# khimansusinha/Distributed-sorting-with-fault-tolerance

Measured on AMD Instinct MI355X. Metric: sorted keys/sec (int32, 2^30 keys), higher is better.
Workload: dtype int32; 1 GPU; C2-style single-GPU sort of 1073741824 uniform int32 keys (BASELINE metric size); tile 8192 keys, 0 merge passes; keys=1073741824, parallelism=1 GPU

## Files before the change

### distributed-sorting-with-fault-tolerance_amd/csrc/dsort_bucket.h

```cpp
#pragma once
#include <hip/hip_runtime.h>
#include <stdint.h>

#include <type_traits>

#include "dsort_internal.h"

namespace dsort {
namespace bk {

constexpr int BK_T = 1024;
constexpr int BK_MAXB = 1024;
constexpr int BK_OS = 32;
constexpr int BK_CHUNK = 16;
constexpr int BK_CSEG = 16;

template <typename T> struct Geo;
template <> struct Geo<int32_t> { static constexpr int KPT = 16; };
constexpr int BK_KPT64 = 6;
template <> struct Geo<int64_t> { static constexpr int KPT = BK_KPT64; };
typedef int bk_v4i __attribute__((ext_vector_type(4)));
typedef long long bk_v2l __attribute__((ext_vector_type(2)));
template <typename T> struct BkIds {
    static constexpr bool ON = sizeof(T) == 8;
// ... 58 lines not shown
template <typename T>
__device__ __forceinline__ int bucket_of(const typename Comp<T>::C *spl, int BP,
                                         const typename Comp<T>::C &c) {
    int lo = 0;
    for (int st = BP >> 1; st >= 1; st >>= 1) lo += Comp<T>::lt(spl[lo + st - 1], c) ? st : 0;
    return lo;
}

constexpr int BK_SLOTB = 11;
constexpr int BK_SLOTS = 1 << BK_SLOTB;

struct BkMap {
    uint64_t ulo;
    uint32_t sh;
    uint32_t mode;
    uint64_t invn;
    uint32_t ids;
    uint32_t hot;
    uint32_t one;
    uint32_t ad;
    uint32_t r2s;
    uint32_t r2lo;
    uint32_t r2sh;
};
constexpr int BK_R2 = 256;
constexpr int BK_R2_BITS = 8;
constexpr uint32_t BK_R2_IMPLIED = 0x4000u;
constexpr size_t BK_MAP_BYTES = 64 + 4 * BK_R2;
static_assert(sizeof(BkMap) <= 64, "the refined table sits 64 bytes into the map");
__host__ __device__ __forceinline__ const uint32_t *bk_tab2(const BkMap *m) {
    return reinterpret_cast<const uint32_t *>(reinterpret_cast<const char *>(m) + 64);
}
constexpr uint32_t BK_PACKED_R2 = 0xFFFFFu;
constexpr uint32_t BK_R2_FLAG = 0x4000u;

template <typename T>
__device__ __forceinline__ uint32_t bucket_runs_hint(uint32_t nasc, uint32_t ndup, int nsp) {
    if (nsp < 16) return 0;
    const uint32_t pairs = (uint32_t)(nsp - 1);
    (void)ndup;
    return (8 * nasc >= 7 * pairs || 8 * nasc <= pairs) ? 1u : 0u;
}
template <bool RANK>
__device__ __forceinline__ uint32_t bucket_bump(uint32_t *hist, int b, bool act) {
    const uint64_t am = __ballot(act);
    if (!am) return 0u;
    const int lane = (int)(threadIdx.x & 63), first = (int)__ffsll((long long)am) - 1;
// ... 179 lines not shown
        if (in == 3) return bucket_onekey<T>(spl, lo, hi, key, c);
        while (lo < hi) {
            const int mid = (lo + hi) >> 1;
            if (Comp<T>::lt(spl[mid], c)) lo = mid + 1;
            else hi = mid;
        }
        return lo;
    }
    if constexpr (!ADP) {
        if (ONE && tab2 && (r & BK_R2_FLAG))
            return refine_pick<T>(spl, tab2[refine_sub(m->r2lo, m->r2sh, (int32_t)key)], key, c);
    }
    int lo = (int)(r & 0x3FFF), hi = (int)(r >> 16);
    if (ONE && (r & 0x8000)) return bucket_onekey<T>(spl, lo, hi, key, c);
    while (lo < hi) {
        const int mid = (lo + hi) >> 1;
        if (Comp<T>::lt(spl[mid], c)) lo = mid + 1;
        else hi = mid;
    }
    return lo;
}

template <typename T>
__global__ void __launch_bounds__(BK_MAXB) bucket_slotmap_kernel(const typename Comp<T>::C *__restrict__ spl,
                                                                  int B, uint64_t n, BkMap *__restrict__ out) {
    using CT = Comp<T>;
    using U = typename CT::U;
    __shared__ uint32_t cnt[2][BK_SLOTS];
    __shared__ uint32_t crowd[2];
    const int j = threadIdx.x, nsp = B - 1;
    for (int i = j; i < 2 * BK_SLOTS; i += blockDim.x) cnt[i / BK_SLOTS][i % BK_SLOTS] = 0;
    if (j < 2) crowd[j] = 0;
    __shared__ uint32_t dup;
    __shared__ uint32_t nasc, ndup;
    if (j == 0) dup = nasc = ndup = 0;
    __syncthreads();
    if (j + 1 < nsp) {
        if (CT::idx_of(spl[j]) < CT::idx_of(spl[j + 1])) atomicAdd(&nasc, 1u);
        if (CT::key_of(spl[j]) == CT::key_of(spl[j + 1])) atomicAdd(&ndup, 1u);
    }
    const uint64_t invn = ((uint64_t)1 << 48) / (n > 0 ? n : 1);
    BkMap mm[2] = {{0, (uint32_t)(CT::KB - BK_SLOTB), 0, invn, 0, 0}, {0, 0, 1, invn, 0, 0}};
    if constexpr (!CT::ADAPT) {
        constexpr uint32_t AD_MIX = 8;
        __shared__ uint32_t tot[3][BK_SLOTS], dst[3][BK_SLOTS];
        __shared__ uint32_t cost[3];
        for (int i = j; i < 3 * BK_SLOTS; i += blockDim.x) tot[i / BK_SLOTS][i % BK_SLOTS] = dst[i / BK_SLOTS][i % BK_SLOTS] = 0;
        if (j < 3) cost[j] = 0;
// ... 17 lines not shown
                if (first) atomicAdd(&dst[q][sl[q]], 1u);
            }
        }
        __syncthreads();
        for (int i = j; i < 3 * BK_SLOTS; i += blockDim.x)
            if (dst[i / BK_SLOTS][i % BK_SLOTS] >= 2) atomicMax(&cost[i / BK_SLOTS], tot[i / BK_SLOTS][i % BK_SLOTS]);
        __syncthreads();
        __shared__ uint32_t r2slot, cost2;
        __shared__ BkMap rm;
        if (j == 0) {
            r2slot = ~0u;
            cost2 = 0;
        }
        __syncthreads();
        const int qa = cost[2] < cost[1] ? 2 : 1;
        if (cost[0] > AD_MIX && cost[qa] > AD_MIX)
            for (int i = j; i < BK_SLOTS; i += blockDim.x)
                if (dst[0][i] >= 2 && tot[0][i] == cost[0]) atomicMin(&r2slot, (uint32_t)i);
        __syncthreads();
        if (r2slot != ~0u)
            for (int i = j; i < BK_SLOTS; i += blockDim.x)
                if ((uint32_t)i != r2slot && dst[0][i] >= 2) atomicMax(&cost2, tot[0][i]);
        __syncthreads();
        const bool refine = r2slot != ~0u && cost2 <= cost[qa];
        const bool fixed = cost[0] <= AD_MIX || refine;
        if (j == 0) {
            if (!refine) r2slot = ~0u;
            BkMap r = fixed ? am[0] : am[qa];
            r.ad = r.ulo != 0 || r.mode != 0 || r.sh != (uint32_t)(CT::KB - BK_SLOTB) ? 1u : 0u;
            r.ids = 0;
            r.hot = bucket_runs_hint<T>(nasc, ndup, nsp);
            r.one = r.ad ? 1u : (ndup != 0);
            r.r2s = r.r2lo = r.r2sh = 0;
            if (r2slot != ~0u) {
                uint32_t a = 0, z = 0;
                for (int k = 0; k < nsp; ++k) {
                    const uint32_t sk = slot_mode<T, BK_SLOTB, 0, false>(am[0], CT::key_of(spl[k]));
                    a += sk < r2slot;
                    z += sk <= r2slot;
                }
                uint64_t us0 = 0;
                (void)slot_first<T, BK_SLOTB>(am[0], r2slot, us0);
                const uint32_t k0 = CT::flip(CT::key_of(spl[a])), hi = CT::flip(CT::key_of(spl[z - 1 - (z - a) / 32]));
                const uint32_t lo = r2slot > 0 && k0 > (uint32_t)us0 ? k0 - 1 : k0;
                const uint32_t rr = hi - lo;
                const int bits = rr == 0 ? 0 : 32 - __builtin_clz(rr);
                r.r2s = r2slot + 1;
                r.r2lo = lo;
                r.r2sh = (uint32_t)(bits > BK_R2_BITS ? bits - BK_R2_BITS : 0);
                r.one = 1;
                static_assert(BK_R2 == 1 << BK_R2_BITS, "sub-slots");
// ... 16 lines not shown
                    const uint32_t mid = (lo + hi) >> 1;
                    if (CT::lt(spl[mid], cc)) lo = mid + 1;
                    else hi = mid;
                }
                return lo;
            };
            (void)BPl;
            const uint32_t c_lo = s2 == 0 ? 0u : below(us), c_hi = has_next ? below(ue) : (uint32_t)nsp;
            for (int i = j; i < BK_R2; i += blockDim.x) {
                uint32_t c0 = c_lo, c1 = c_hi;
                if (i > 0) {
                    const uint64_t u = (uint64_t)rm.r2lo + ((uint64_t)i << rm.r2sh);
                    c0 = has_next && u >= ue ? c_hi : (u > 0xFFFFFFFFull ? c_hi : below(u));
                }
                if (i + 1 < BK_R2) {
                    const uint64_t u = (uint64_t)rm.r2lo + ((uint64_t)(i + 1) << rm.r2sh);
                    c1 = has_next && u >= ue ? c_hi : (u > 0xFFFFFFFFull ? c_hi : below(u));
                }
                c0 = c0 < c_lo ? c_lo : c0;
                const bool one = c1 >= c0 + 2 && CT::key_of(spl[c0]) == CT::key_of(spl[c1 - 1]);
                const bool implied = rm.r2sh == 0 && i > 0 && i + 1 < BK_R2;
                tab[i] = c0 | (implied ? BK_R2_IMPLIED : 0u) | (uint32_t)one << 15 | c1 << 16;
            }
        }
        return;
    }
    if (nsp >= 1) {
        const U lo = CT::flip(CT::key_of(spl[0])), hi = CT::flip(CT::key_of(spl[nsp - 1]));
        const U r = hi - lo;
        const int bits = r == 0 ? 0 : (int)(sizeof(U) * 8) - (sizeof(U) == 8 ? __builtin_clzll((uint64_t)r)
                                                                               : __builtin_clz((uint32_t)r));
        mm[0] = BkMap{(uint64_t)lo, (uint32_t)(bits > BK_SLOTB ? bits - BK_SLOTB : 0), 0, invn, 0, 0};
        mm[1] = BkMap{(uint64_t)lo, 0, 1, invn, 0, 0};
    }
    __syncthreads();
    if (j > 0 && j < nsp && CT::key_of(spl[j]) == CT::key_of(spl[j - 1])) dup = 1;
    if (j < nsp && (j == 0 || CT::key_of(spl[j]) != CT::key_of(spl[j - 1]))) {
        const T k = CT::key_of(spl[j]);
        atomicAdd(&cnt[0][slot_at<T>(mm[0], k)], 1u);
        atomicAdd(&cnt[1][slot_at<T>(mm[1], k)], 1u);
    }
    __syncthreads();
    for (int i = j; i < 2 * BK_SLOTS; i += blockDim.x) atomicMax(&crowd[i / BK_SLOTS], cnt[i / BK_SLOTS][i % BK_SLOTS]);
    __syncthreads();
    if (j == 0) {
        BkMap r = crowd[1] < crowd[0] ? mm[1] : mm[0];
// ... 81 lines not shown

constexpr uint64_t BK_CUS = 256;
template <typename T>
__host__ __forceinline__ int bucket_wg_subs(uint64_t n) {
    const uint64_t sub = (uint64_t)BK_T * Geo<T>::KPT;
    const uint64_t v = n / (2048 * sub);
    const int cap = v < 4 ? 4 : (v > 16 ? 16 : (int)v);
    if (cap > 4) {
        const uint64_t nsub = (n + sub - 1) / sub;
        int best = cap;
        uint64_t bcost = ~0ull;
        for (int s = cap; s >= (cap + 1) / 2; --s) {
            const uint64_t rounds = ((nsub + s - 1) / s + BK_CUS - 1) / BK_CUS;
            if (rounds * s < bcost) {
                bcost = rounds * s;
                best = s;
            }
        }
        return best;
    }
    return cap;
}

template <typename T, bool AD = false>
__global__ void __launch_bounds__(BK_T, 2) bucket_hist_kernel(const T *__restrict__ in, uint64_t n,
                                                              const typename Comp<T>::C *__restrict__ spl_g,
                                                              const BkMap *__restrict__ map, int B, int BP,
                                                              int subs, uint32_t *__restrict__ counts,
                                                              uint64_t ioff, uint32_t *__restrict__ ids) {
    using CT = Comp<T>;
    constexpr bool ADP = CT::ADAPT || AD;
    constexpr int KPT = Geo<T>::KPT, SUB = BK_T * KPT;
    static_assert(!BkIds<T>::ON || KPT % BkIds<T>::PER_WORD == 0, "bucket ids: whole words per thread");
    __shared__ typename CT::C spl[BK_MAXB + 1];
    __shared__ uint32_t rng[BK_SLOTS];
    const BkMap m = *map;
    if (!ADP && m.ad) return;
    __shared__ uint32_t hist[BK_MAXB];
    __shared__ uint32_t tab2[ADP ? 1 : BK_R2];
    load_splitters<T>(spl_g, BP, spl);
    for (int b = threadIdx.x; b < B; b += BK_T) hist[b] = 0;
    if (!ADP && m.r2s)
        for (int i = threadIdx.x; i < BK_R2; i += BK_T) tab2[i] = bk_tab2(map)[i];
    __syncthreads();
    build_slots<T, false, BK_SLOTB, ADP>(spl, BP, m, rng);
    __syncthreads();
    const uint64_t g0 = (uint64_t)blockIdx.x * subs * SUB;
    T nxt[KPT];
    load_sub<T, KPT, false>(in, g0 + threadIdx.x, n, g0 + SUB, nxt);
#pragma unroll 1
    for (int sub = 0; sub < subs; ++sub) {
        const uint64_t b0 = g0 + (uint64_t)sub * SUB + threadIdx.x;
        T key[KPT];
#pragma unroll
        for (int k = 0; k < KPT; ++k) key[k] = nxt[k];
        if (sub + 1 < subs) load_sub<T, KPT, false>(in, b0 + SUB, n, b0 - threadIdx.x + 2 * SUB, nxt);
        constexpr int PW = BkIds<T>::PER_WORD;
        uint32_t idw[BkIds<T>::ON ? KPT / PW : 1] = {};
        const auto idput = [&](int k, int b) {
            if constexpr (BkIds<T>::ON) idw[k / PW] |= (uint32_t)b << (BkIds<T>::BITS * (k % PW));
        };
        if (m.hot) {
#pragma unroll
            for (int k = 0; k < KPT; ++k) {
                const uint64_t i = b0 + (uint64_t)k * BK_T;
                const uint32_t sl = m.mode == 0 ? slot_mode<T, BK_SLOTB, 0, ADP>(m, key[k]) : slot_mode<T, BK_SLOTB, 1, ADP>(m, key[k]);
                const int b = bucket_fast<T, false, true, ADP>(spl, rng, sl, key[k], CT::make(key[k], i + ioff), tab2, &m);
                bucket_bump<false>(hist, b, i < n);
                if (i < n) idput(k, b);
            }
        } else if (ADP ? m.mode == 0 : !m.one) {
#pragma unroll
// ... 181 lines not shown
    }
}


template <typename T> struct LineGeo {
    static constexpr int LK = 64 / (int)sizeof(T);
    static constexpr int KPL = 16 / (int)sizeof(T);
    static constexpr int SUB = BK_T * Geo<T>::KPT;
    static constexpr int MAPN = (SUB + 2 * (LK - 1) * BK_MAXB) / LK;
};
#ifdef DSORT_STAMPS
__device__ unsigned long long g_bkstamps[8192 * 16];
#define BKST(k)                                            \
    do {                                                   \
        const uint64_t t1_ = __builtin_amdgcn_s_memtime(); \
        bk_acc[k] += t1_ - bk_t0;                          \
        bk_t0 = t1_;                                       \
    } while (0)
#else
#define BKST(k) \
    do {        \
    } while (0)
#endif
template <typename T, bool IDS, bool AD = false, bool HT = false>
__global__ void __launch_bounds__(BK_T) bucket_scatter_lines_kernel(const T *__restrict__ in, uint64_t n,
                                                                    const typename Comp<T>::C *__restrict__ spl_g,
                                                                    const BkMap *__restrict__ map, int B, int BP, int subs,
                                                                    const uint32_t *__restrict__ offs,
                                                                    T *__restrict__ out, T *__restrict__ out2,
                                                                    uint64_t ioff, const uint32_t *__restrict__ ids) {
    using CT = Comp<T>;
    constexpr bool ADP = CT::ADAPT || AD;
    static_assert(!IDS || BkIds<T>::ON, "bucket ids of this key width");
    using G = LineGeo<T>;
    using V = typename std::conditional<sizeof(T) == 4, int4, longlong2>::type;
    constexpr int KPT = Geo<T>::KPT, SUB = G::SUB, LK = G::LK, KPL = G::KPL;
    static_assert(SUB + LK < (1 << 16) && LK <= 16, "packed fields");
    constexpr bool SPL_LK = !CT::ADAPT;
    __shared__ typename CT::C spl_own[SPL_LK || IDS ? 1 : BK_MAXB + 1];
    __shared__ uint32_t rng[IDS ? 1 : BK_SLOTS];
    __shared__ uint32_t hist[BK_MAXB];
    __shared__ uint2 st[BK_MAXB];
    __shared__ uint32_t sgb[BK_MAXB];
    __shared__ uint16_t lmap[G::MAPN];
    __shared__ uint32_t wsum[BK_T / 64];
    __shared__ T lk[SUB];
    __shared__ T carry[BK_MAXB * LK];
    static_assert(!SPL_LK || sizeof(lk) >= (BK_MAXB + 1) * sizeof(typename CT::C), "splitters staged in lk");
    const auto cswz = [](uint32_t b, uint32_t e) { return e ^ ((b >> 1) & (uint32_t)(LK - 1)); };
    typename CT::C *spl = SPL_LK ? reinterpret_cast<typename CT::C *>(lk) : spl_own;
    const typename CT::C *spl_look = SPL_LK ? spl_g : spl;
    const int tb = threadIdx.x, lane = tb & 63, w = tb >> 6;
    const uint32_t g = blockIdx.x;
    const bool owner = tb < B;
    uint32_t vc = 0, ph = 0, gb = 0, pure = 0;
    if (owner) {
        const uint32_t o = offs[(uint64_t)g * B + tb];
        pure = out2 && tb > 0 && tb + 1 < B && CT::key_of(spl_g[tb - 1]) == CT::key_of(spl_g[tb]);
        ph = (uint32_t)(((uintptr_t)((pure ? out2 : out) + o) / sizeof(T)) & (LK - 1));
        vc = ph;
        gb = o - ph;
        hist[tb] = 0;
    }
    __shared__ uint32_t pmask[BK_MAXB / 32];
    {
        const uint64_t pb = __ballot(pure != 0);
        if (lane == 0 && 2 * w + 1 < BK_MAXB / 32) {
            pmask[2 * w] = (uint32_t)pb;
            pmask[2 * w + 1] = (uint32_t)(pb >> 32);
        }
    }
    const BkMap m = *map;
    __shared__ uint32_t tab2s[ADP || IDS ? 1 : BK_R2];
    const uint32_t *tab2 = ADP || IDS ? nullptr : tab2s;
    if (BkIds<T>::ON && (m.ids != 0) != IDS) return;
    if (!IDS) {
        load_splitters<T>(spl_g, BP, spl);
        if (!ADP && m.r2s)
            for (int i = tb; i < BK_R2; i += BK_T) tab2s[i] = bk_tab2(map)[i];
        __syncthreads();
        build_slots<T, true, BK_SLOTB, ADP>(spl, BP, m, rng);
    }
    __syncthreads();
    bool anyp = false;
#pragma unroll
    for (int i = 0; i < BK_MAXB / 32; ++i) anyp = anyp || pmask[i] != 0u;
    const auto dropped = [&](int b) { return anyp && ((pmask[b >> 5] >> (b & 31)) & 1u) != 0u; };
    const uint64_t g0 = (uint64_t)g * subs * SUB;
#ifdef DSORT_STAMPS
    uint64_t bk_acc[8] = {}, bk_t0 = __builtin_amdgcn_s_memtime();
#endif
    T nxt[KPT];
    constexpr int PW = BkIds<T>::PER_WORD;
    uint32_t nid[IDS ? KPT / PW : 1];
    const auto load_ids = [&](uint64_t s) {
        if constexpr (IDS) {
            const uint32_t *src = ids + s / SUB * (KPT / PW) * BK_T + tb;
#pragma unroll
            for (int w = 0; w < KPT / PW; ++w) nid[w] = src[w * BK_T];
        }
    };
    load_sub<T, KPT>(in, g0 + tb, n, g0 + SUB, nxt);
    if constexpr (IDS) {
        if (g0 < n) load_ids(g0);
    }
#pragma unroll 1
    for (int sub = 0; sub < subs; ++sub) {
        const uint64_t s0 = g0 + (uint64_t)sub * SUB;
        if (s0 >= n) break;
        const bool last = sub + 1 == subs || s0 + SUB >= n;
        T key[KPT];
        uint32_t pk[KPT];
        uint32_t sl[KPT];
#pragma unroll
        for (int k = 0; k < KPT; ++k) key[k] = nxt[k];
        if constexpr (IDS) {
#pragma unroll
            for (int k = 0; k < KPT; ++k) sl[k] = (nid[k / PW] >> (BkIds<T>::BITS * (k % PW))) & BkIds<T>::MASK;
        } else {
            slots_at<T, KPT, ADP>(m, key, sl);
        }
        if (!last) {
            load_sub<T, KPT>(in, s0 + SUB + tb, n, s0 + 2 * SUB, nxt);
            if constexpr (IDS) load_ids(s0 + SUB);
        }
        BKST(6);
        if (m.hot) {
#pragma unroll
            for (int k = 0; k < KPT; ++k) {
                const uint64_t i = s0 + tb + (uint64_t)k * BK_T;
                const bool act = i < n;
                const int b = IDS ? (int)sl[k] : bucket_fast<T, true, true, ADP>(spl_look, rng, sl[k], key[k], CT::make(key[k], i + ioff), tab2, &m);
                const bool a = act && !dropped(b);
                const uint32_t r = bucket_bump<true>(hist, b, a);
                pk[k] = a ? r | (uint32_t)b << 16 : ~0u;
            }
        } else {
          bool batched = false;
          if constexpr (!ADP && !IDS) {
           if (s0 + SUB <= n) {
            batched = true;
            constexpr int CB = 4;
#pragma unroll
            for (int k0 = 0; k0 < KPT; k0 += CB) {
                uint32_t r[CB];
                int b[CB];
                bool sw[CB], any = false;
#pragma unroll
                for (int g = 0; g < CB; ++g) r[g] = rng[sl[k0 + g]];
#pragma unroll
// ... 140 lines not shown
```

### distributed-sorting-with-fault-tolerance_amd/csrc/dsort_internal.h

```cpp
#pragma once

#include <hip/hip_runtime.h>
#include <stdint.h>
#include <stddef.h>

#include <atomic>
#include <mutex>
#include <string>
#include <utility>
#include <vector>

#include "dsort.h"

struct ncclComm;
namespace dsort {
class TxSeq;
}

namespace dsort {

constexpr int kMaxLogF = 5;
constexpr int kMaxF = 1 << kMaxLogF;

struct GroupK {
// ... 90 lines not shown
}

struct dsort_opts {
    int64_t buckets = -1;
    int64_t bucket_keys = 1 << 20;
    static constexpr int64_t BUCKET_OS_DEFAULT = 128;
    int64_t bucket_os = BUCKET_OS_DEFAULT;
    int64_t max_logf = -1;
    int64_t kill_after_pass = -1;
    int64_t stage_timing = 1;
    int64_t kill_in_exchange = -1;
    int64_t comm_timeout_ms = 0;
    int64_t test_hold_exchange = 0;
    int64_t test_fail_exchange = -1;
    int64_t test_tile_cap = 0;
    int64_t test_wave_fence = 0;
    int64_t sub_keys = -1;
    int64_t sub_os = -1;
    int64_t sub_gather = 1;
    int64_t argsort_wide = 0;
    int64_t test_fail_leg = -1;
    int64_t topk_path = -1;
    int64_t sub_arith = -1;
};

struct dsort_ctx {
    using DevBuf = dsort::DevBuf;
    using HostBuf = dsort::HostBuf;
    using Event = dsort::Event;
    using Stream = dsort::Stream;
    using LegClock = dsort::LegClock;

    dsort_opts opt;
    int nested = 0;
    int stages_done = 0;
    std::atomic<int> abort_req{0};
    std::mutex comm_mu;
    int device = 0;
    std::string err;

    Stream stream;
    Stream side;
    Stream xs;

    Event groups_ev;
    Event bucket_ev;
// ... 58 lines not shown
    bool done_pending = false;
    DevBuf tfb;
    DevBuf text_status;
    DevBuf red;
    HostBuf red_host;
    ncclComm *comm = nullptr;
    bool has_transport = false;
    dsort_transport transport = {};
    dsort::TxSeq *tx = nullptr;
    HostBuf xfer;
    HostBuf xfer2;
    DevBuf fence;
    HostBuf fence_host;
    int nranks = 1;
    int rank = 0;
    DevBuf local;
    DevBuf recv;
    DevBuf recv2;
    DevBuf small;
    HostBuf small_host;
    DevBuf bxs;
    const uint32_t *bk_hot = nullptr;
    uint32_t sub_arith_n[2] = {0, 0};
    int ev_off = 0;
    int ev_done = dsort::kEvLocalDone;
    bool poll_waits = false;
    double poll_deadline = 0.0;
    hipStream_t poll_stream = nullptr;
    std::vector<void *> dev_later, host_later;
    uint64_t deferred_n = 0;
    unsigned ev_mask = 0;
    hipStream_t last_stream = nullptr;
    int kev_used = 0;
    bool ev_ok = false;
    bool ev_created = false;
    dsort_stats stats = {};
};

namespace dsort {

__device__ __forceinline__ uint32_t wave_incl_sum(uint32_t v) {
    v += (uint32_t)__builtin_amdgcn_update_dpp(0, (int)v, 0x111, 0xF, 0xF, false);
    v += (uint32_t)__builtin_amdgcn_update_dpp(0, (int)v, 0x112, 0xF, 0xF, false);
    v += (uint32_t)__builtin_amdgcn_update_dpp(0, (int)v, 0x114, 0xF, 0xF, false);
    v += (uint32_t)__builtin_amdgcn_update_dpp(0, (int)v, 0x118, 0xF, 0xF, false);
    v += (uint32_t)__builtin_amdgcn_update_dpp(0, (int)v, 0x142, 0xA, 0xF, false);
// ... 83 lines not shown
```

### distributed-sorting-with-fault-tolerance_amd/csrc/dsort_sub.h

```cpp
#pragma once
#include <hip/hip_runtime.h>
#include <stdint.h>

#include "dsort_bucket.h"

namespace dsort {
namespace sb {

constexpr int SB_T = 256;
constexpr int SB_MAXS = 1024;
constexpr int SB_SLOTB = 10;
constexpr int SB_SLOTS = 1 << SB_SLOTB;
constexpr int SB_ST = 4;
template <typename T> constexpr int SB_KPT = sizeof(T) == 4 ? 16 : 8;
template <typename T> constexpr int SB_SUB = SB_T * SB_KPT<T>;
template <typename T> constexpr int SB_CH = SB_ST * SB_SUB<T>;

struct BInfo {
    uint64_t start;
    uint64_t soff;
    uint32_t len;
    uint32_t nsub;
    uint32_t ns;
    uint32_t c0, c1;
// ... 37 lines not shown
    T klo;
    uint32_t sh;
    uint32_t scale;
};

template <typename T>
__host__ __device__ __forceinline__ uint32_t slot_of(T key, T klo, uint32_t sh) {
    using U = typename KeyU<T>::U;
    const U d = key < klo ? (U)0 : (U)((U)key - (U)klo);
    const U s = d >> sh;
    return s > (U)(SB_SLOTS - 1) ? (uint32_t)(SB_SLOTS - 1) : (uint32_t)s;
}

template <typename T> struct Spl;
template <> struct __attribute__((aligned(8))) Spl<int32_t> {
    int32_t k;
    uint32_t p;
};
template <> struct __attribute__((aligned(16))) Spl<int64_t> {
    int64_t k;
    uint32_t p, pad;
};

template <typename T> constexpr bool SB_ARITH = sizeof(T) == 4;
__host__ __device__ __forceinline__ bool arith_span_ok(uint32_t span, uint32_t nsub) { return span >= 2 * nsub; }
__host__ __device__ __forceinline__ uint32_t arith_scale(uint32_t span, uint32_t nsub) {
    return (uint32_t)(((uint64_t)nsub << 32) / ((uint64_t)span + 1));
}
__host__ __device__ __forceinline__ uint32_t arith_sub(int32_t key, int32_t klo, uint32_t scale, uint32_t nsub) {
    const uint32_t d = key < klo ? 0u : (uint32_t)key - (uint32_t)klo;
    const uint32_t j = (uint32_t)(((uint64_t)d * scale) >> 32);
    return j < nsub - 1 ? j : nsub - 1;
}
__host__ __device__ __forceinline__ int32_t arith_splitter_key(int32_t klo, uint32_t scale, uint32_t j) {
    const uint64_t d = ((((uint64_t)j + 1) << 32) + scale - 1) / scale - 1;
    const int64_t k = (int64_t)klo + (int64_t)d;
    return k < (int64_t)INT32_MAX ? (int32_t)k : INT32_MAX;
}
constexpr uint32_t SB_ARITH_MAXS = 3;
constexpr uint32_t SB_ARITH_MAXS_RUNS = 6;

template <typename T>
__host__ __device__ __forceinline__ bool below(const Spl<T> &s, T key, uint32_t pos) {
    return s.k < key || (s.k == key && s.p <= pos);
}

constexpr uint32_t SB_ONEKEY = 0x8000u;
template <typename T>
__host__ __device__ __forceinline__ int sub_pick(const Spl<T> *spl, uint32_t r, const Spl<T> &a, const Spl<T> &b, T key,
                                        uint32_t pos) {
    int lo = (int)(r & 0x7FFF);
    const int hi = (int)(r >> 16);
    if (r & SB_ONEKEY) {
        if (key != a.k) return key < a.k ? lo : hi;
        if (pos < a.p) return lo;
        const Spl<T> z = spl[hi - 1];
        if (pos >= z.p) return hi;
        const float f = (float)((pos * 2654435761u) >> 8) * 0x1p-24f;
        const int jj = (int)(f * (float)(hi - lo - 1));
        return lo + 1 + (jj < hi - lo - 2 ? jj : hi - lo - 2);
// ... 903 lines not shown
```

### distributed-sorting-with-fault-tolerance_amd/csrc/dsort_wave.hip

```cpp
#include <hip/hip_runtime.h>

#include <stdint.h>

#include <algorithm>
#include <climits>
#include <ctime>
#include <sched.h>
#include <unistd.h>
#include <csignal>
#include <cstdlib>
#include <cstring>
#include <string>
#include <type_traits>
#include <vector>

#include "dsort_bucket.h"
#include "dsort_internal.h"
#include "dsort_tx.h"

#include <rocprofiler-sdk-roctx/roctx.h>
#include "dsort_part.h"
#include "dsort_sub.h"

namespace dsort {
// ... 1983 lines not shown
    L.cnt = reinterpret_cast<uint32_t *>(a + o_cnt);
    L.part = reinterpret_cast<uint64_t *>(a + o_part);
    L.offs = reinterpret_cast<uint32_t *>(a + o_offs);
    L.bst = reinterpret_cast<uint64_t *>(a + o_bst);
    L.cst = reinterpret_cast<uint64_t *>(a + o_cst);
    L.tt = reinterpret_cast<TileRef *>(a + o_tt);
    L.ntl = reinterpret_cast<uint32_t *>(a + o_nt);
    L.map = reinterpret_cast<BkMap *>(a + o_map);
    L.ids = BkIds<T>::ON ? reinterpret_cast<uint32_t *>(a + o_ids) : nullptr;
    const size_t hbytes = (size_t)(BK_MAXB + 1) * 8 + (size_t)BK_MAXB * 16 + sizeof(BkMap);
    if (ctx->bucket_host.bytes < hbytes) {
        release_host(ctx, ctx->bucket_host);
        DSORT_HIP(ctx, hipHostMalloc(&ctx->bucket_host.p, hbytes, hipHostMallocDefault));
        ctx->bucket_host.bytes = hbytes;
    }
    if (!ctx->bucket_ev && hipEventCreateWithFlags(&ctx->bucket_ev.h, hipEventDisableTiming) != hipSuccess)
        return set_err(ctx, DSORT_EHIP, "hipEventCreate");
    return DSORT_OK;
}

template <typename T>
static int first_level(dsort_ctx *ctx, const T *d_in, uint64_t n, uint64_t ioff, T *part_out, T *direct,
                       const BkLayout<T> &L, uint32_t tile, hipStream_t s, bool timed, uint64_t *&hb,
                       typename bk::Comp<T>::C *&hspl, bool compact = false) {
    using namespace bk;
    using C = typename Comp<T>::C;
    const int B = L.B, BP = L.BP;
    int rc;
    hb = ctx->bucket_host.as<uint64_t>();
    hspl = reinterpret_cast<C *>(hb + BK_MAXB + 1);
    hipLaunchKernelGGL(bucket_slotmap_kernel<T>, dim3(1), dim3(BK_MAXB), 0, s, L.spl, B, n, L.map);
    ctx->bk_hot = &L.map->hot;
    BkMap *hm = reinterpret_cast<BkMap *>(reinterpret_cast<char *>(hb) + (size_t)(BK_MAXB + 1) * 8 + (size_t)BK_MAXB * 16);
    DSORT_HIP(ctx, hipMemcpyAsync(hm, L.map, sizeof(BkMap), hipMemcpyDeviceToHost, s));
    DSORT_HIP(ctx, hipEventRecord(ctx->bucket_ev, s));
    if ((rc = stage_event(ctx, s, timed, kEvHist0))) return rc;
    hipLaunchKernelGGL((bucket_hist_kernel<T, false>), dim3((unsigned)L.G), dim3(BK_T), 0, s, d_in, n, L.spl, L.map, B,
                       BP, L.subs, L.cnt, ioff, L.ids);
    if (int rc_ = sync_event(ctx, ctx->bucket_ev, "slot map")) return rc_;
    const bool ad = !Comp<T>::ADAPT && hm->ad != 0, ids = BkIds<T>::ON && hm->ids != 0;
    if constexpr (!Comp<T>::ADAPT) {
        if (ad)
            hipLaunchKernelGGL((bucket_hist_kernel<T, true>), dim3((unsigned)L.G), dim3(BK_T), 0, s, d_in, n, L.spl,
                               L.map, B, BP, L.subs, L.cnt, ioff, L.ids);
    }
    if ((rc = stage_event(ctx, s, timed, kEvHist1))) return rc;
    hipLaunchKernelGGL(bucket_colsum_kernel, dim3((unsigned)L.nchunk), dim3(BK_MAXB), 0, s, L.cnt, (uint32_t)L.G, B,
                       L.part);
    uint64_t *ctot = L.part + (size_t)L.nchunk * B;
    hipLaunchKernelGGL(bucket_colscan_kernel, dim3((unsigned)ceil_div((uint64_t)B, 64)), dim3(BK_MAXB), 0, s, L.part,
                       (uint32_t)L.nchunk, B, ctot);
    hipLaunchKernelGGL(bucket_scan_kernel<T>, dim3(1), dim3(BK_MAXB), 0, s, L.part, (uint32_t)L.nchunk, B, tile,
                       (uint32_t)KPC<T>, L.bst, L.tt, L.ntl, (const uint64_t *)ctot, compact ? L.spl : nullptr, L.cst);
    hipLaunchKernelGGL(bucket_offsets_kernel<uint32_t>, dim3((unsigned)L.nchunk), dim3(BK_MAXB), 0, s, L.cnt, L.part,
                       compact ? L.cst : L.bst, (uint32_t)L.G, B, L.offs);
    if (compact) direct = part_out;
    DSORT_HIP(ctx, hipGetLastError());
    if ((rc = side_stream(ctx))) return rc;
    DSORT_HIP(ctx, hipEventRecord(ctx->ready_ev, s));
    DSORT_HIP(ctx, hipStreamWaitEvent(ctx->side, ctx->ready_ev, 0));
    DSORT_HIP(ctx, hipMemcpyAsync(hb, L.bst, (size_t)(B + 1) * 8, hipMemcpyDeviceToHost, ctx->side));
    if (B > 1) DSORT_HIP(ctx, hipMemcpyAsync(hspl, L.spl, (size_t)(B - 1) * sizeof(C), hipMemcpyDeviceToHost, ctx->side));
    DSORT_HIP(ctx, hipEventRecord(ctx->bucket_ev, ctx->side));
    if ((rc = stage_event(ctx, s, timed, kEvScatter0))) return rc;
    if constexpr (!Comp<T>::ADAPT) {
        if (ad)
            hipLaunchKernelGGL((bucket_scatter_lines_kernel<T, false, true>), dim3((unsigned)L.G), dim3(BK_T), 0, s,
                               d_in, n, L.spl, L.map, B, BP, L.subs, L.offs, part_out, direct, ioff, L.ids);
    }
    if (!ad && !ids) {
        if (!Comp<T>::ADAPT && hm->hot)
            hipLaunchKernelGGL((bucket_scatter_lines_kernel<T, false, false, true>), dim3((unsigned)L.G), dim3(BK_T), 0,
                               s, d_in, n, L.spl, L.map, B, BP, L.subs, L.offs, part_out, direct, ioff, L.ids);
        else
            hipLaunchKernelGGL((bucket_scatter_lines_kernel<T, false, false>), dim3((unsigned)L.G), dim3(BK_T), 0, s,
                               d_in, n, L.spl, L.map, B, BP, L.subs, L.offs, part_out, direct, ioff, L.ids);
    }
    if constexpr (BkIds<T>::ON)
        if (ids)
            hipLaunchKernelGGL((bucket_scatter_lines_kernel<T, true>), dim3((unsigned)L.G), dim3(BK_T), 0, s, d_in, n,
                               L.spl, L.map, B, BP, L.subs, L.offs, part_out, direct, ioff, L.ids);
    DSORT_HIP(ctx, hipGetLastError());
    if ((rc = stage_event(ctx, s, timed, kEvScatter1))) return rc;
    fault_point(ctx, s, 0);
    if (int rc_ = sync_event(ctx, ctx->bucket_ev, "bucket starts")) return rc_;
    if (hb[B] != n) return set_err(ctx, DSORT_EHIP, "bucket partition lost keys");
    ctx->stats.first_level_map = !Comp<T>::ADAPT && !ad ? (hm->r2s ? 3 : 0) : hm->mode == 0 ? 1 : 2;
    return DSORT_OK;
}

static int bucketed_stats_start(dsort_ctx *ctx, uint64_t n, int tile, hipStream_t s, bool timed) {
    ctx->bk_hot = nullptr;
    ctx->sub_arith_n[0] = ctx->sub_arith_n[1] = 0;
    ctx->stats = fresh_stats();
    ctx->stats.keys_in = ctx->stats.keys_out = n;
    ctx->stats.tile_sort_keys = n;
    ctx->stats.tile_keys = tile;
    ctx->ev_mask = 0;
    ctx->kev_used = 0;
    ctx->last_stream = s;
    return stage_event(ctx, s, timed, kEvStart);
}

template <typename T>
static int bucket_sort(dsort_ctx *ctx, const T *d_in, T *d_keys, size_t n, hipStream_t s, bool timed, int B) {
    using namespace bk;
    using C = typename Comp<T>::C;
    constexpr int TILE = TILE_OF<T>;
    constexpr uint64_t ALIGN = KPC<T>;
    const int os = bucket_os(ctx);
    const uint32_t S = (uint32_t)B * (uint32_t)os;
    BkLayout<T> L;
    int rc = bk_layout<T>(ctx, n, B, (size_t)S * (sizeof(T) == 8 ? 24 : sizeof(C)), L);
    if (rc) return rc;
    const int BP = L.BP;
    C *smp = reinterpret_cast<C *>(L.smp);
// ... 12 lines not shown
                                             : set_err(ctx, DSORT_EHIP, "bucket_sample_kernel launch");
    } else {
        hipLaunchKernelGGL(pair_sample_keys_kernel, dim3(ceil_div(S, 256)), dim3(256), 0, s, d_in, (uint64_t)n, pk, S);
        rc = sort_device<int64_t>(ctx, pk, psrt, S, s, false);
        if (!rc) {
            hipLaunchKernelGGL(pair_rank_kernel, dim3(ceil_div(S, 256)), dim3(256), 0, s, pk, psrt, S, pcmp);
            rc = sort_device<int64_t>(ctx, pcmp, pcmp, S, s, false);
        }
    }
    --ctx->nested;
    if (rc) return rc;
    if ((rc = bucketed_stats_start(ctx, n, TILE, s, timed))) return rc;
    if constexpr (std::is_same<T, int32_t>::value) {
        hipLaunchKernelGGL(bucket_splitter_kernel<int32_t>, dim3(1), dim3(BK_MAXB), 0, s, smp, B, BP, os, spl);
    } else {
        hipLaunchKernelGGL(pair_splitter_kernel, dim3(1), dim3(BK_MAXB), 0, s, pcmp, pk, (uint64_t)n, S, B, BP, os,
                           spl);
    }
    T *part_out = scratch;
    T *direct = sub_keys<T>(ctx) && (const void *)d_in != (const void *)d_keys && n < (1ull << 31) ? d_keys : nullptr;
    uint64_t *hb;
    C *hspl;
    rc = first_level<T>(ctx, d_in, n, 0, part_out, direct, L, sub_keys<T>(ctx) ? 0u : (uint32_t)TILE, s, timed, hb,
                        hspl);
    if (rc) return rc;
    if (const uint64_t m = sub_keys<T>(ctx)) {
        std::vector<uint8_t> pure((size_t)B, 0);
        for (int b = 1; b + 1 < B; ++b) pure[b] = Comp<T>::key_of(hspl[b - 1]) == Comp<T>::key_of(hspl[b]);
        std::vector<T> fk;
        if (direct) {
            fk.assign((size_t)B, T(0));
            for (int b = 1; b + 1 < B; ++b)
                if (pure[b]) fk[b] = Comp<T>::key_of(hspl[b]);
        }
        return sub_sort<T>(ctx, part_out, d_keys, n, hb, B, m, s, timed, ctx->opt.sub_gather != 0, pure.data(),
                           direct != nullptr, spl, nullptr, fk.empty() ? nullptr : fk.data());
    }
    std::vector<std::vector<uint64_t>> runs(B);
    uint64_t maxruns = 1;
    for (int b = 0; b < B; ++b) {
        const uint64_t len = hb[b + 1] - hb[b], h = bucket_head(hb[b], len, ALIGN);
        if (h) runs[b].push_back(h);
        for (uint64_t o = h; o < len; o += TILE) runs[b].push_back(len - o < (uint64_t)TILE ? len - o : TILE);
        maxruns = runs[b].size() > maxruns ? runs[b].size() : maxruns;
    }
    const std::vector<int> pbits = plan_passes<T>(ctx->opt, maxruns);
    const int passes = (int)pbits.size();
// ... 498 lines not shown
        rc = launch_pass_w<T, false>(ctx, src, dst, pd, logf, tiles, s, !keep_stats);
        if (rc) return rc;
        rl.swap(next);
        src = dst;
        which ^= 1;
    }
    return DSORT_OK;
}

}

extern "C" int dsort_debug_sub_arith_mode(dsort_ctx *ctx, int mode) {
    if (!ctx || (mode != -1 && mode != 0 && mode != 2)) return DSORT_EINVAL;
    ctx->opt.sub_arith = mode;
    return DSORT_OK;
}
extern "C" int dsort_debug_sub_arith(const dsort_ctx *ctx, uint32_t out[2]) {
    if (!ctx || !out) return DSORT_EINVAL;
    out[0] = ctx->sub_arith_n[0];
    out[1] = ctx->sub_arith_n[1];
    return DSORT_OK;
}

#ifdef DSORT_STAMPS
extern "C" int dsort_debug_stamps(void *host, size_t bytes) {
    return hipMemcpyFromSymbol(host, HIP_SYMBOL(wv::g_stamps), bytes) == hipSuccess ? 0 : -1;
}
extern "C" int dsort_debug_bkstamps(void *host, size_t bytes) {
    return hipMemcpyFromSymbol(host, HIP_SYMBOL(bk::g_bkstamps), bytes) == hipSuccess ? 0 : -1;
}
extern "C" int dsort_debug_sbstamps(void *host, size_t bytes) {
    return hipMemcpyFromSymbol(host, HIP_SYMBOL(sb::g_sbstamps), bytes) == hipSuccess ? 0 : -1;
}
#endif

void PollPause::operator()() {
    const double t = tx_now_ms();
    if (t0 < 0) t0 = t;
    if (t - t0 < POLL_SPIN_MS) sched_yield();
    else usleep(20);
}
static int poll_done(dsort_ctx *ctx, hipError_t (*query)(void *), void *h, const char *what, bool comm) {
    PollPause pause;
    for (;;) {
        const hipError_t q = query(h);
        if (q == hipSuccess) return DSORT_OK;
// ... 91 lines not shown
```

### distributed-sorting-with-fault-tolerance_amd/dsort.py

```python
import contextlib
import ctypes
import os

import numpy as np

HERE = os.path.dirname(os.path.abspath(__file__))
LIB_PATH = os.environ.get("DSORT_LIB") or os.path.join(HERE, "lib", "libdsort.so")

try:
    import torch
except Exception:
    torch = None

DSORT_OK = 0
DSORT_ECOMM = -4
DSORT_ETIMEOUT = -6
ERRORS = {-1: "EINVAL", -2: "ENOMEM", -3: "EHIP", -4: "ECOMM", -5: "ENODEV", -6: "ETIMEOUT", -7: "ESTAGE"}

EXPORTS = [
    "dsort_init", "dsort_finalize", "dsort_last_error", "dsort_version", "dsort_get_stats",
    "dsort_synchronize", "dsort_set_option", "dsort_get_option", "dsort_sort_stages", "dsort_sample_sort_stages", "dsort_sort_i32", "dsort_sort_i64", "dsort_sort_dev_i32",
    "dsort_sort_dev_i64", "dsort_sort_dev_copy_i32", "dsort_sort_dev_copy_i64",
    "dsort_merge_i32", "dsort_merge_i64", "dsort_merge_dev_i32", "dsort_merge_dev_i64",
    "dsort_comm_unique_id", "dsort_comm_init", "dsort_comm_init_transport", "dsort_comm_abort",
# ... 450 lines not shown
    def _opt(name):
        return OPTIONS[name]

    def set_option(self, name, value):
        self.check(self.lib.dsort_set_option(self.h, self._opt(name), int(value)))

    def get_option(self, name):
        v = ctypes.c_int64()
        self.check(self.lib.dsort_get_option(self.h, self._opt(name), ctypes.byref(v)))
        return v.value

    def sub_arith_mode(self, mode):
        f = self.lib.dsort_debug_sub_arith_mode
        f.restype, f.argtypes = ctypes.c_int, [P, ctypes.c_int]
        self.check(f(self.h, int(mode)))

    def sub_arith_counts(self):
        out = (ctypes.c_uint32 * 2)()
        f = self.lib.dsort_debug_sub_arith
        f.restype, f.argtypes = ctypes.c_int, [P, P]
        self.check(f(self.h, ctypes.cast(out, P)))
        return int(out[0]), int(out[1])

    @contextlib.contextmanager
    def options(self, **kw):
        old = {k: self.get_option(k) for k in kw}
        try:
            for k, v in kw.items():
                self.set_option(k, v)
            yield self
        finally:
            for k, v in old.items():
                self.set_option(k, v)

    def sort_stages(self, n, key_bytes=4):
        m = ctypes.c_int()
        self.check(self.lib.dsort_sort_stages(self.h, n, key_bytes, ctypes.byref(m)))
        return m.value

    def sort(self, keys, descending=False, key_type=None):
        assert keys.flags.c_contiguous
        name = _np_key(keys, key_type)
        if name in ("i32", "i64") and not descending:
            f = getattr(self.lib, f"dsort_sort_{name}")
            self.check(f(self.h, _ptr(keys), keys.size))
        else:
# ... 418 lines not shown
```

Measured before the change: 147.7 billion keys/s.

## Use arithmetic bucket mapping for first-level partition of uniform int32 keys

Adds an arithmetic first-level bucket map for int32 keys. The bucket is computed as (key-lo)*scale>>32, which replaces the splitter slot lookup and binary search in the histogram and scatter kernels. The slotmap kernel checks each bucket's sample load against the oversampling factor, falls back to the splitter path when any bucket would be overfull, and rewrites the splitters so later stages stay consistent. This cuts per-key compute and shared-memory table setup, but risks imbalance on skewed data if the sample check misses it.

After: 151.4 billion keys/s (median of 6 runs). +2.5%, better.

```diff
diff --git a/distributed-sorting-with-fault-tolerance_amd/csrc/dsort_bucket.h b/distributed-sorting-with-fault-tolerance_amd/csrc/dsort_bucket.h
--- a/distributed-sorting-with-fault-tolerance_amd/csrc/dsort_bucket.h
+++ b/distributed-sorting-with-fault-tolerance_amd/csrc/dsort_bucket.h
@@ -104,7 +104,32 @@
     uint32_t r2s;
     uint32_t r2lo;
     uint32_t r2sh;
+    uint32_t ar;
+    uint32_t arlo;
+    uint32_t arscale;
 };
+
+template <typename T> constexpr bool BK_ARITH = sizeof(T) == 4;
+__host__ __device__ __forceinline__ bool arith_span_ok(uint32_t span, uint32_t n) { return span >= 2 * n; }
+__host__ __device__ __forceinline__ uint32_t arith_scale(uint32_t span, uint32_t n) {
+    return (uint32_t)(((uint64_t)n << 32) / ((uint64_t)span + 1));
+}
+__host__ __device__ __forceinline__ uint32_t arith_part(int32_t key, int32_t klo, uint32_t scale, uint32_t n) {
+    const uint32_t d = key < klo ? 0u : (uint32_t)key - (uint32_t)klo;
+    const uint32_t j = (uint32_t)(((uint64_t)d * scale) >> 32);
+    return j < n - 1 ? j : n - 1;
+}
+__host__ __device__ __forceinline__ int32_t arith_splitter_key(int32_t klo, uint32_t scale, uint32_t j) {
+    const uint64_t d = ((((uint64_t)j + 1) << 32) + scale - 1) / scale - 1;
+    const int64_t k = (int64_t)klo + (int64_t)d;
+    return k < (int64_t)INT32_MAX ? (int32_t)k : INT32_MAX;
+}
+__host__ __device__ __forceinline__ int arith_bucket(int32_t key, const BkMap &m, int B) {
+    return (int)arith_part(key, (int32_t)m.arlo, m.arscale, (uint32_t)B);
+}
+__host__ __device__ __forceinline__ bool arith_bucket_full(uint32_t samples, uint32_t os) {
+    return 2 * (uint64_t)samples > 3 * (uint64_t)os;
+}
 constexpr int BK_R2 = 256;
 constexpr int BK_R2_BITS = 8;
 constexpr uint32_t BK_R2_IMPLIED = 0x4000u;
@@ -330,8 +355,10 @@
 }
 
 template <typename T>
-__global__ void __launch_bounds__(BK_MAXB) bucket_slotmap_kernel(const typename Comp<T>::C *__restrict__ spl,
-                                                                  int B, uint64_t n, BkMap *__restrict__ out) {
+__global__ void __launch_bounds__(BK_MAXB) bucket_slotmap_kernel(typename Comp<T>::C *spl, int B, uint64_t n,
+                                                                  BkMap *__restrict__ out,
+                                                                  const typename Comp<T>::C *smp, uint32_t ns, int os,
+                                                                  int arith) {
     using CT = Comp<T>;
     using U = typename CT::U;
     __shared__ uint32_t cnt[2][BK_SLOTS];
@@ -395,11 +422,50 @@
             for (int i = j; i < BK_SLOTS; i += blockDim.x)
                 if ((uint32_t)i != r2slot && dst[0][i] >= 2) atomicMax(&cost2, tot[0][i]);
         __syncthreads();
-        const bool refine = r2slot != ~0u && cost2 <= cost[qa];
-        const bool fixed = cost[0] <= AD_MIX || refine;
+        const bool refine_s = r2slot != ~0u && cost2 <= cost[qa];
+        const bool fixed_s = cost[0] <= AD_MIX || refine_s;
+        __shared__ uint32_t ar_ub[BK_MAXB];
+        __shared__ uint32_t ar_bad;
+        bool ar_on = false;
+        int32_t ar_klo = 0;
+        uint32_t ar_scale = 0;
+        if constexpr (BK_ARITH<T>) {
+            if (smp && arith != 0 && ns > 0 && B >= 2) {
+                ar_klo = CT::key_of(smp[0]);
+                const uint32_t span = (uint32_t)CT::key_of(smp[ns - 1]) - (uint32_t)ar_klo;
+                const bool plain = fixed_s && !refine_s && ndup == 0 && !bucket_runs_hint<T>(nasc, ndup, nsp);
+                if (arith_span_ok(span, (uint32_t)B) && (arith > 0 || plain)) {
+                    ar_scale = arith_scale(span, (uint32_t)B);
+                    ar_on = true;
+                }
+            }
+            if (ar_on && arith < 0) {
+                if (j == 0) ar_bad = 0;
+                uint32_t ub = ns;
+                if (j < B - 1) {
+                    const int32_t K = arith_splitter_key(ar_klo, ar_scale, (uint32_t)j);
+                    uint32_t lo = 0, hi = ns;
+                    while (lo < hi) {
+                        const uint32_t mid = (lo + hi) >> 1;
+                        if (CT::key_of(smp[mid]) <= K) lo = mid + 1;
+                        else hi = mid;
+                    }
+                    ub = lo;
+                }
+                if (j < B) ar_ub[j] = ub;
+                __syncthreads();
+                if (j < B && arith_bucket_full(ub - (j ? ar_ub[j - 1] : 0u), (uint32_t)os)) ar_bad = 1;
+                __syncthreads();
+                if (ar_bad) ar_on = false;
+            }
+        }
+        const bool refine = refine_s && !ar_on, fixed = fixed_s || ar_on;
         if (j == 0) {
             if (!refine) r2slot = ~0u;
             BkMap r = fixed ? am[0] : am[qa];
+            r.ar = ar_on ? 1u : 0u;
+            r.arlo = (uint32_t)ar_klo;
+            r.arscale = ar_on ? ar_scale : 0u;
             r.ad = r.ulo != 0 || r.mode != 0 || r.sh != (uint32_t)(CT::KB - BK_SLOTB) ? 1u : 0u;
             r.ids = 0;
             r.hot = bucket_runs_hint<T>(nasc, ndup, nsp);
@@ -462,6 +528,9 @@
                 const bool implied = rm.r2sh == 0 && i > 0 && i + 1 < BK_R2;
                 tab[i] = c0 | (implied ? BK_R2_IMPLIED : 0u) | (uint32_t)one << 15 | c1 << 16;
             }
+        }
+        if constexpr (BK_ARITH<T>) {
+            if (rm.ar && j < nsp) spl[j] = CT::make(arith_splitter_key((int32_t)rm.arlo, rm.arscale, (uint32_t)j), 0xFFFFFFFFull);
         }
         return;
     }
@@ -589,7 +658,7 @@
     return cap;
 }
 
-template <typename T, bool AD = false>
+template <typename T, bool AD = false, bool AR = false>
 __global__ void __launch_bounds__(BK_T, 2) bucket_hist_kernel(const T *__restrict__ in, uint64_t n,
                                                               const typename Comp<T>::C *__restrict__ spl_g,
                                                               const BkMap *__restrict__ map, int B, int BP,
@@ -599,22 +668,46 @@
     constexpr bool ADP = CT::ADAPT || AD;
     constexpr int KPT = Geo<T>::KPT, SUB = BK_T * KPT;
     static_assert(!BkIds<T>::ON || KPT % BkIds<T>::PER_WORD == 0, "bucket ids: whole words per thread");
-    __shared__ typename CT::C spl[BK_MAXB + 1];
-    __shared__ uint32_t rng[BK_SLOTS];
+    static_assert(!AR || (BK_ARITH<T> && !AD), "the arithmetic map: int32 on the plain fixed map");
+    __shared__ typename CT::C spl[AR ? 1 : BK_MAXB + 1];
+    __shared__ uint32_t rng[AR ? 1 : BK_SLOTS];
     const BkMap m = *map;
-    if (!ADP && m.ad) return;
+    if (!ADP && !AR && (m.ad || m.ar)) return;
     __shared__ uint32_t hist[BK_MAXB];
     __shared__ uint32_t tab2[ADP ? 1 : BK_R2];
-    load_splitters<T>(spl_g, BP, spl);
+    if constexpr (!AR) load_splitters<T>(spl_g, BP, spl);
     for (int b = threadIdx.x; b < B; b += BK_T) hist[b] = 0;
     if (!ADP && m.r2s)
         for (int i = threadIdx.x; i < BK_R2; i += BK_T) tab2[i] = bk_tab2(map)[i];
     __syncthreads();
-    build_slots<T, false, BK_SLOTB, ADP>(spl, BP, m, rng);
-    __syncthreads();
+    if constexpr (!AR) {
+        build_slots<T, false, BK_SLOTB, ADP>(spl, BP, m, rng);
+        __syncthreads();
+    }
     const uint64_t g0 = (uint64_t)blockIdx.x * subs * SUB;
     T nxt[KPT];
     load_sub<T, KPT, false>(in, g0 + threadIdx.x, n, g0 + SUB, nxt);
+    if constexpr (AR) {
+#pragma unroll 1
+        for (int sub = 0; sub < subs; ++sub) {
+            const uint64_t b0 = g0 + (uint64_t)sub * SUB + threadIdx.x;
+            int bb[KPT];
+#pragma unroll
+            for (int k = 0; k < KPT; ++k) bb[k] = arith_bucket((int32_t)nxt[k], m, B);
+            if (sub + 1 < subs) load_sub<T, KPT, false>(in, b0 + SUB, n, b0 - threadIdx.x + 2 * SUB, nxt);
+            if (b0 - threadIdx.x + SUB <= n) {
+#pragma unroll
+                for (int k = 0; k < KPT; ++k) atomicAdd(&hist[bb[k]], 1u);
+            } else {
+#pragma unroll
+                for (int k = 0; k < KPT; ++k)
+                    if (b0 + (uint64_t)k * BK_T < n) atomicAdd(&hist[bb[k]], 1u);
+            }
+        }
+        __syncthreads();
+        for (int b = threadIdx.x; b < B; b += BK_T) counts[(uint64_t)blockIdx.x * B + b] = hist[b];
+        return;
+    }
 #pragma unroll 1
     for (int sub = 0; sub < subs; ++sub) {
         const uint64_t b0 = g0 + (uint64_t)sub * SUB + threadIdx.x;
@@ -842,7 +935,7 @@
     do {        \
     } while (0)
 #endif
-template <typename T, bool IDS, bool AD = false, bool HT = false>
+template <typename T, bool IDS, bool AD = false, bool HT = false, bool AR = false>
 __global__ void __launch_bounds__(BK_T) bucket_scatter_lines_kernel(const T *__restrict__ in, uint64_t n,
                                                                     const typename Comp<T>::C *__restrict__ spl_g,
                                                                     const BkMap *__restrict__ map, int B, int BP, int subs,
@@ -852,13 +945,14 @@
     using CT = Comp<T>;
     constexpr bool ADP = CT::ADAPT || AD;
     static_assert(!IDS || BkIds<T>::ON, "bucket ids of this key width");
+    static_assert(!AR || (BK_ARITH<T> && !IDS && !AD && !HT), "the arithmetic map: int32 on the plain fixed map");
     using G = LineGeo<T>;
     using V = typename std::conditional<sizeof(T) == 4, int4, longlong2>::type;
     constexpr int KPT = Geo<T>::KPT, SUB = G::SUB, LK = G::LK, KPL = G::KPL;
     static_assert(SUB + LK < (1 << 16) && LK <= 16, "packed fields");
     constexpr bool SPL_LK = !CT::ADAPT;
     __shared__ typename CT::C spl_own[SPL_LK || IDS ? 1 : BK_MAXB + 1];
-    __shared__ uint32_t rng[IDS ? 1 : BK_SLOTS];
+    __shared__ uint32_t rng[IDS || AR ? 1 : BK_SLOTS];
     __shared__ uint32_t hist[BK_MAXB];
     __shared__ uint2 st[BK_MAXB];
     __shared__ uint32_t sgb[BK_MAXB];
@@ -891,10 +985,10 @@
         }
     }
     const BkMap m = *map;
-    __shared__ uint32_t tab2s[ADP || IDS ? 1 : BK_R2];
-    const uint32_t *tab2 = ADP || IDS ? nullptr : tab2s;
+    __shared__ uint32_t tab2s[ADP || IDS || AR ? 1 : BK_R2];
+    const uint32_t *tab2 = ADP || IDS || AR ? nullptr : tab2s;
     if (BkIds<T>::ON && (m.ids != 0) != IDS) return;
-    if (!IDS) {
+    if (!IDS && !AR) {
         load_splitters<T>(spl_g, BP, spl);
         if (!ADP && m.r2s)
             for (int i = tb; i < BK_R2; i += BK_T) tab2s[i] = bk_tab2(map)[i];
@@ -937,6 +1031,9 @@
         if constexpr (IDS) {
 #pragma unroll
             for (int k = 0; k < KPT; ++k) sl[k] = (nid[k / PW] >> (BkIds<T>::BITS * (k % PW))) & BkIds<T>::MASK;
+        } else if constexpr (AR) {
+#pragma unroll
+            for (int k = 0; k < KPT; ++k) sl[k] = (uint32_t)arith_bucket((int32_t)key[k], m, B);
         } else {
             slots_at<T, KPT, ADP>(m, key, sl);
         }
@@ -945,7 +1042,21 @@
             if constexpr (IDS) load_ids(s0 + SUB);
         }
         BKST(6);
-        if (m.hot) {
+        if constexpr (AR) {
+            if (s0 + SUB <= n && !anyp) {
+#pragma unroll
+                for (int k = 0; k < KPT; ++k) pk[k] = atomicAdd(&hist[sl[k]], 1u);
+#pragma unroll
+                for (int k = 0; k < KPT; ++k) pk[k] |= sl[k] << 16;
+            } else {
+#pragma unroll
+                for (int k = 0; k < KPT; ++k) {
+                    const uint64_t i = s0 + tb + (uint64_t)k * BK_T;
+                    pk[k] = ~0u;
+                    if (i < n && !dropped((int)sl[k])) pk[k] = atomicAdd(&hist[sl[k]], 1u) | sl[k] << 16;
+                }
+            }
+        } else if (m.hot) {
 #pragma unroll
             for (int k = 0; k < KPT; ++k) {
                 const uint64_t i = s0 + tb + (uint64_t)k * BK_T;
diff --git a/distributed-sorting-with-fault-tolerance_amd/csrc/dsort_internal.h b/distributed-sorting-with-fault-tolerance_amd/csrc/dsort_internal.h
--- a/distributed-sorting-with-fault-tolerance_amd/csrc/dsort_internal.h
+++ b/distributed-sorting-with-fault-tolerance_amd/csrc/dsort_internal.h
@@ -136,6 +136,7 @@
     int64_t test_fail_leg = -1;
     int64_t topk_path = -1;
     int64_t sub_arith = -1;
+    int64_t bk_arith = -1;
 };
 
 struct dsort_ctx {
@@ -240,6 +241,7 @@
     DevBuf bxs;
     const uint32_t *bk_hot = nullptr;
     uint32_t sub_arith_n[2] = {0, 0};
+    uint32_t bk_arith_on = 0;
     int ev_off = 0;
     int ev_done = dsort::kEvLocalDone;
     bool poll_waits = false;
diff --git a/distributed-sorting-with-fault-tolerance_amd/csrc/dsort_sub.h b/distributed-sorting-with-fault-tolerance_amd/csrc/dsort_sub.h
--- a/distributed-sorting-with-fault-tolerance_amd/csrc/dsort_sub.h
+++ b/distributed-sorting-with-fault-tolerance_amd/csrc/dsort_sub.h
@@ -83,20 +83,12 @@
     uint32_t p, pad;
 };
 
-template <typename T> constexpr bool SB_ARITH = sizeof(T) == 4;
-__host__ __device__ __forceinline__ bool arith_span_ok(uint32_t span, uint32_t nsub) { return span >= 2 * nsub; }
-__host__ __device__ __forceinline__ uint32_t arith_scale(uint32_t span, uint32_t nsub) {
-    return (uint32_t)(((uint64_t)nsub << 32) / ((uint64_t)span + 1));
-}
+template <typename T> constexpr bool SB_ARITH = bk::BK_ARITH<T>;
+using bk::arith_scale;
+using bk::arith_span_ok;
+using bk::arith_splitter_key;
 __host__ __device__ __forceinline__ uint32_t arith_sub(int32_t key, int32_t klo, uint32_t scale, uint32_t nsub) {
-    const uint32_t d = key < klo ? 0u : (uint32_t)key - (uint32_t)klo;
-    const uint32_t j = (uint32_t)(((uint64_t)d * scale) >> 32);
-    return j < nsub - 1 ? j : nsub - 1;
-}
-__host__ __device__ __forceinline__ int32_t arith_splitter_key(int32_t klo, uint32_t scale, uint32_t j) {
-    const uint64_t d = ((((uint64_t)j + 1) << 32) + scale - 1) / scale - 1;
-    const int64_t k = (int64_t)klo + (int64_t)d;
-    return k < (int64_t)INT32_MAX ? (int32_t)k : INT32_MAX;
+    return bk::arith_part(key, klo, scale, nsub);
 }
 constexpr uint32_t SB_ARITH_MAXS = 3;
 constexpr uint32_t SB_ARITH_MAXS_RUNS = 6;
diff --git a/distributed-sorting-with-fault-tolerance_amd/csrc/dsort_wave.hip b/distributed-sorting-with-fault-tolerance_amd/csrc/dsort_wave.hip
--- a/distributed-sorting-with-fault-tolerance_amd/csrc/dsort_wave.hip
+++ b/distributed-sorting-with-fault-tolerance_amd/csrc/dsort_wave.hip
@@ -2029,14 +2029,17 @@
 template <typename T>
 static int first_level(dsort_ctx *ctx, const T *d_in, uint64_t n, uint64_t ioff, T *part_out, T *direct,
                        const BkLayout<T> &L, uint32_t tile, hipStream_t s, bool timed, uint64_t *&hb,
-                       typename bk::Comp<T>::C *&hspl, bool compact = false) {
+                       typename bk::Comp<T>::C *&hspl, bool compact = false, bool arith = false) {
     using namespace bk;
     using C = typename Comp<T>::C;
     const int B = L.B, BP = L.BP;
     int rc;
     hb = ctx->bucket_host.as<uint64_t>();
     hspl = reinterpret_cast<C *>(hb + BK_MAXB + 1);
-    hipLaunchKernelGGL(bucket_slotmap_kernel<T>, dim3(1), dim3(BK_MAXB), 0, s, L.spl, B, n, L.map);
+    const bool ar_ok = BK_ARITH<T> && arith;
+    hipLaunchKernelGGL(bucket_slotmap_kernel<T>, dim3(1), dim3(BK_MAXB), 0, s, L.spl, B, n, L.map,
+                       ar_ok ? reinterpret_cast<const C *>(L.smp) : (const C *)nullptr,
+                       (uint32_t)B * (uint32_t)bucket_os(ctx), bucket_os(ctx), ar_ok ? (int)ctx->opt.bk_arith : 0);
     ctx->bk_hot = &L.map->hot;
     BkMap *hm = reinterpret_cast<BkMap *>(reinterpret_cast<char *>(hb) + (size_t)(BK_MAXB + 1) * 8 + (size_t)BK_MAXB * 16);
     DSORT_HIP(ctx, hipMemcpyAsync(hm, L.map, sizeof(BkMap), hipMemcpyDeviceToHost, s));
@@ -2050,6 +2053,9 @@
         if (ad)
             hipLaunchKernelGGL((bucket_hist_kernel<T, true>), dim3((unsigned)L.G), dim3(BK_T), 0, s, d_in, n, L.spl,
                                L.map, B, BP, L.subs, L.cnt, ioff, L.ids);
+        else if (BK_ARITH<T> && hm->ar)
+            hipLaunchKernelGGL((bucket_hist_kernel<T, false, BK_ARITH<T>>), dim3((unsigned)L.G), dim3(BK_T), 0, s, d_in,
+                               n, L.spl, L.map, B, BP, L.subs, L.cnt, ioff, L.ids);
     }
     if ((rc = stage_event(ctx, s, timed, kEvHist1))) return rc;
     hipLaunchKernelGGL(bucket_colsum_kernel, dim3((unsigned)L.nchunk), dim3(BK_MAXB), 0, s, L.cnt, (uint32_t)L.G, B,
@@ -2075,7 +2081,15 @@
             hipLaunchKernelGGL((bucket_scatter_lines_kernel<T, false, true>), dim3((unsigned)L.G), dim3(BK_T), 0, s,
                                d_in, n, L.spl, L.map, B, BP, L.subs, L.offs, part_out, direct, ioff, L.ids);
     }
-    if (!ad && !ids) {
+    bool ar = false;
+    if constexpr (BK_ARITH<T>) {
+        ar = !ad && hm->ar != 0;
+        if (ar)
+            hipLaunchKernelGGL((bucket_scatter_lines_kernel<T, false, false, false, true>), dim3((unsigned)L.G),
+                               dim3(BK_T), 0, s, d_in, n, L.spl, L.map, B, BP, L.subs, L.offs, part_out, direct, ioff,
+                               L.ids);
+    }
+    if (!ad && !ids && !ar) {
         if (!Comp<T>::ADAPT && hm->hot)
             hipLaunchKernelGGL((bucket_scatter_lines_kernel<T, false, false, true>), dim3((unsigned)L.G), dim3(BK_T), 0,
                                s, d_in, n, L.spl, L.map, B, BP, L.subs, L.offs, part_out, direct, ioff, L.ids);
@@ -2093,12 +2107,14 @@
     if (int rc_ = sync_event(ctx, ctx->bucket_ev, "bucket starts")) return rc_;
     if (hb[B] != n) return set_err(ctx, DSORT_EHIP, "bucket partition lost keys");
     ctx->stats.first_level_map = !Comp<T>::ADAPT && !ad ? (hm->r2s ? 3 : 0) : hm->mode == 0 ? 1 : 2;
+    ctx->bk_arith_on = ar ? 1u : 0u;
     return DSORT_OK;
 }
 
 static int bucketed_stats_start(dsort_ctx *ctx, uint64_t n, int tile, hipStream_t s, bool timed) {
     ctx->bk_hot = nullptr;
     ctx->sub_arith_n[0] = ctx->sub_arith_n[1] = 0;
+    ctx->bk_arith_on = 0;
     ctx->stats = fresh_stats();
     ctx->stats.keys_in = ctx->stats.keys_out = n;
     ctx->stats.tile_sort_keys = n;
@@ -2157,7 +2173,7 @@
     uint64_t *hb;
     C *hspl;
     rc = first_level<T>(ctx, d_in, n, 0, part_out, direct, L, sub_keys<T>(ctx) ? 0u : (uint32_t)TILE, s, timed, hb,
-                        hspl);
+                        hspl, false, std::is_same<T, int32_t>::value);
     if (rc) return rc;
     if (const uint64_t m = sub_keys<T>(ctx)) {
         std::vector<uint8_t> pure((size_t)B, 0);
@@ -2702,6 +2718,17 @@
     return DSORT_OK;
 }
 
+extern "C" int dsort_debug_bucket_arith_mode(dsort_ctx *ctx, int mode) {
+    if (!ctx || (mode != -1 && mode != 0 && mode != 2)) return DSORT_EINVAL;
+    ctx->opt.bk_arith = mode;
+    return DSORT_OK;
+}
+extern "C" int dsort_debug_bucket_arith(const dsort_ctx *ctx, uint32_t out[1]) {
+    if (!ctx || !out) return DSORT_EINVAL;
+    out[0] = ctx->bk_arith_on;
+    return DSORT_OK;
+}
+
 #ifdef DSORT_STAMPS
 extern "C" int dsort_debug_stamps(void *host, size_t bytes) {
     return hipMemcpyFromSymbol(host, HIP_SYMBOL(wv::g_stamps), bytes) == hipSuccess ? 0 : -1;
diff --git a/distributed-sorting-with-fault-tolerance_amd/dsort.py b/distributed-sorting-with-fault-tolerance_amd/dsort.py
--- a/distributed-sorting-with-fault-tolerance_amd/dsort.py
+++ b/distributed-sorting-with-fault-tolerance_amd/dsort.py
@@ -496,6 +496,18 @@
         self.check(f(self.h, ctypes.cast(out, P)))
         return int(out[0]), int(out[1])
 
+    def bucket_arith_mode(self, mode):
+        f = self.lib.dsort_debug_bucket_arith_mode
+        f.restype, f.argtypes = ctypes.c_int, [P, ctypes.c_int]
+        self.check(f(self.h, int(mode)))
+
+    def bucket_arith(self):
+        out = (ctypes.c_uint32 * 1)()
+        f = self.lib.dsort_debug_bucket_arith
+        f.restype, f.argtypes = ctypes.c_int, [P, P]
+        self.check(f(self.h, ctypes.cast(out, P)))
+        return bool(out[0])
+
     @contextlib.contextmanager
     def options(self, **kw):
         old = {k: self.get_option(k) for k in kw}
```
